# TinfoilHat0/Defending-Against-Backdoors-with-Robust-Learning-Rate

Hardware: NVIDIA H100
Metric: fl_rounds_per_sec (higher is better)
Workload: dtype bf16

## Files before the change

### defending-against-backdoors-with-robust-learning-rate_b200/ops/csrc/gemm.cu

```cuda
#include <cuda.h>
#include <stdlib.h>

#include "common.cuh"
#include "gemm.h"
#include "stem_gather.cuh"
#include "wgmma.cuh"

namespace rlr {

using namespace wg;

constexpr int BM = 128;
constexpr int BK = 64;
constexpr int kConsumers = 256;
constexpr int kThreads = kConsumers + 64;
constexpr int kEpiThreads = kConsumers;

template <int BN, int kOcc = 2>
struct TileCfg {
    static_assert(kOcc != 1 || BN == 128, "the one-wave configuration exists for the 128-wide tile");
    static constexpr int kStages = kOcc == 1 ? 6 : kOcc == 3 ? (BN == 64 ? 3 : 2) : (BN == 64 ? 4 : 3);
    static constexpr int kABytes = BM * BK * 2;
    static constexpr int kBBytes = BN * BK * 2;
    static constexpr int kStageBytes = kABytes + kBBytes;
// ... 3 lines not shown
    static_assert(kStagingBytes + 2 * BN * 4 <= kRingBytes, "staging aliases the operand ring");
    static constexpr int kTailBytes = BN == 128 ? 2048 : 1024;
    static constexpr int kSmemBytes = kRingBytes + 1024  + kTailBytes;
    static_assert(kStages <= 8, "SharedTail holds eight barriers per array");
};

struct __align__(8) SharedTail {
    uint64_t full[8];
    uint64_t empty[8];
    int row_index[BM];
};
static_assert(sizeof(SharedTail) <= 640, "the bias slice starts 640 bytes into the tail");

template <int BN, bool kStats, bool kBMN, int kOcc = 2>
__global__ void __launch_bounds__(kThreads, kOcc)
umma_conv_gemm_kernel(const __grid_constant__ CUtensorMap tmA, const __grid_constant__ CUtensorMap tmB, const __grid_constant__ CUtensorMap tmC,
                       const ConvGemmParams p) {
    using Cfg = TileCfg<BN, kOcc>;
    extern __shared__ uint8_t smem_raw[];
    uint8_t* smem = reinterpret_cast<uint8_t*>((reinterpret_cast<uintptr_t>(smem_raw) + 1023) & ~uintptr_t(1023));
    SharedTail* tail = reinterpret_cast<SharedTail*>(smem + Cfg::kRingBytes);

    const int warp = threadIdx.x >> 5, lane = threadIdx.x & 31;
    const int tile_m = blockIdx.x, tile_n = blockIdx.y;
    long long* dbg = p.dbg ? p.dbg + ((size_t)blockIdx.y * gridDim.x + blockIdx.x) * 8 : nullptr;
    if (dbg && threadIdx.x == 0) { dbg[0] = (long long)gtimer(); uint32_t sm; asm volatile("mov.u32 %0, %%smid;" : "=r"(sm)); dbg[7] = sm; }

    int n0 = 0, h0 = 0, w0 = 0;
    if (p.mode == 1) {
        const int tw_i = tile_m % p.tiles_w;
        const int th_i = (tile_m / p.tiles_w) % p.tiles_h;
        const int tn_i = tile_m / (p.tiles_w * p.tiles_h);
        w0 = tw_i * p.TW; h0 = th_i * p.TH; n0 = tn_i * p.TN;
    }

    if (warp == 8 && lane == 0) {
        prefetch_tmap(&tmA);
        prefetch_tmap(&tmB);
        if (p.tma_store) prefetch_tmap(&tmC);
        for (int s = 0; s < Cfg::kStages; ++s) { mbar_init(&tail->full[s], (p.split_prod || p.b_src) ? 2 : 1); mbar_init(&tail->empty[s], 8); }
        fence_barrier_init();
    }
    if (threadIdx.x < BM) {
        const int r = threadIdx.x;
        int gi;
        if (p.mode == 1) {
            const int tw = r % p.TW, th = (r / p.TW) % p.TH, tn = r / (p.TW * p.TH);
            const int w = w0 + tw, h = h0 + th, n = n0 + tn;
            gi = (w < p.Wo && h < p.Ho && n < p.NB) ? ((n * p.OutH + h * p.out_stride + p.out_ph) * p.OutW + w * p.out_stride + p.out_pw) : -1;
        } else {
            gi = tile_m * BM + r;
            if (gi >= p.M) gi = -1;
        }
        tail->row_index[r] = gi;
    }
    __syncthreads();
    pdl_wait();
    pdl_trigger();
    if (dbg && threadIdx.x == 0) dbg[1] = (long long)gtimer();

    if (warp == 8) {
        if (p.b_src) {
            if (lane == 0) {
                mbar_expect_tx(&tail->full[0], Cfg::kABytes);
                tma_load_2d(&tmA, &tail->full[0], smem, 0, tile_m * BM);
            }
            stem_gather_b(p, smem + Cfg::kABytes, BN, tile_n, lane);
            if (lane == 0) mbar_arrive(&tail->full[0]);
        } else if (lane == 0) {
            int stage = 0;
            uint32_t phase = 0;
            for (int kb = 0; kb < p.num_kb; ++kb) {
                mbar_wait(&tail->empty[stage], phase ^ 1);
                uint8_t* sa = smem + stage * Cfg::kStageBytes;
                uint8_t* sb = sa + Cfg::kABytes;
                mbar_expect_tx(&tail->full[stage], p.split_prod ? Cfg::kABytes : Cfg::kStageBytes);
                if (dbg && kb == 0) dbg[2] = (long long)gtimer();
                if (p.mode == 1) {
                    const int tap = kb / p.cblocks, cb = kb - tap * p.cblocks;
                    tma_load_4d(&tmA, &tail->full[stage], sa, cb * BK, w0 * p.in_stride + p.dw[tap], h0 * p.in_stride + p.dh[tap],
                                n0 + p.dn[tap]);
                } else {
                    tma_load_2d(&tmA, &tail->full[stage], sa, kb * BK, tile_m * BM);
                }
                if (p.split_prod) {
                } else if (kBMN) {
                    const int tap = kb / p.cblocks, cb = kb - tap * p.cblocks;
                    for (int g = 0; g < BN / 64; ++g)
                        tma_load_2d(&tmB, &tail->full[stage], sb + g * 8192, p.wtap[tap] * p.wcols + tile_n * BN + g * 64, cb * BK);
                } else {
                    tma_load_2d(&tmB, &tail->full[stage], sb, kb * BK, tile_n * BN);
                }
                if (++stage == Cfg::kStages) { stage = 0; phase ^= 1; }
            }
        }
    } else if (warp == 9) {
        if (p.split_prod && lane == 0) {
            int stage = 0;
            uint32_t phase = 0;
            for (int kb = 0; kb < p.num_kb; ++kb) {
                mbar_wait(&tail->empty[stage], phase ^ 1);
                uint8_t* sb = smem + stage * Cfg::kStageBytes + Cfg::kABytes;
                mbar_expect_tx(&tail->full[stage], Cfg::kBBytes);
                if (kBMN) {
                    const int tap = kb / p.cblocks, cb = kb - tap * p.cblocks;
                    for (int g = 0; g < BN / 64; ++g)
                        tma_load_2d(&tmB, &tail->full[stage], sb + g * 8192, p.wtap[tap] * p.wcols + tile_n * BN + g * 64, cb * BK);
                } else {
                    tma_load_2d(&tmB, &tail->full[stage], sb, kb * BK, tile_n * BN);
                }
                if (++stage == Cfg::kStages) { stage = 0; phase ^= 1; }
            }
        }
    } else {
        const int et = threadIdx.x;
        const int wgi = et >> 7, t = et & 127;
        const int col0 = tile_n * BN;
        const bool has_bias = !kBMN && p.bias != nullptr;
        float* bias_w = reinterpret_cast<float*>(reinterpret_cast<uint8_t*>(tail) + 640);
        if (has_bias)
            for (int i = et; i < BN; i += kEpiThreads) bias_w[i] = (col0 + i < p.N) ? p.bias[col0 + i] : 0.f;
        float acc[BN / 2];
#pragma unroll
        for (int i = 0; i < BN / 2; ++i) acc[i] = 0.f;
        {
            int stage = 0;
            uint32_t phase = 0;
            consumer_mainloop<BN, Cfg::kStages, Cfg::kStageBytes, Cfg::kABytes, kBMN>(
                acc, smem, tail->full, tail->empty, p.num_kb, (uint32_t)wgi * 64 * 128, p.b_src ? smem_u32(smem + Cfg::kABytes) : 0u,
                stage, phase, lane);
        }
        if (dbg && et == 0) dbg[4] = (long long)gtimer();
        named_bar(1, kEpiThreads);
        if (dbg && et == 0) dbg[5] = (long long)gtimer();
        const float* bias_s = bias_w;
        uint8_t* staging = smem;
        float* red = reinterpret_cast<float*>(staging + Cfg::kStagingBytes);
        const int r0 = wgi * 64 + frag_row(t, 0);
        int gi_r[2];
        gi_r[0] = tail->row_index[r0];
        gi_r[1] = tail->row_index[r0 + 8];
        if (kStats) {
            for (int i = et; i < 2 * BN; i += kEpiThreads) red[i] = 0.f;
            named_bar(1, kEpiThreads);
        }
        const bool tma_out = !kStats && p.tma_store;
#pragma unroll
        for (int j = 0; j < BN / 8; ++j) {
            const int c = frag_col(t, 4 * j);
            float s1[2] = {0.f, 0.f}, s2[2] = {0.f, 0.f};
#pragma unroll
            for (int h = 0; h < 2; ++h) {
// ... 145 lines not shown
}

template <int BN>
cudaError_t launch_persistent_bn(const CUtensorMap& tmA, const CUtensorMap& tmB, const ConvGemmParams& p, int m_tiles, int num_sms,
                                 cudaStream_t st, int occ = 1);

static int g_occ3 = -1;
void set_conv_occ3(int level) { g_occ3 = level < 0 ? 0 : (level > 1 ? 1 : level); }
static int conv_occ3() {
    if (g_occ3 < 0) { const char* e = getenv("RLR_CONV_OCC3"); set_conv_occ3(e ? atoi(e) : 1); }
    return g_occ3;
}

template <int BN, int kOcc>
static cudaError_t launch_bn_occ(const CUtensorMap& tmA, const CUtensorMap& tmB, const CUtensorMap& tmC, const ConvGemmParams& p, int m_tiles,
                                 cudaStream_t st) {
    using Cfg = TileCfg<BN, kOcc>;
    static bool configured = false;
    if (!configured) {
        RLR_CUDA_CHECK(cudaFuncSetAttribute(umma_conv_gemm_kernel<BN, false, false, kOcc>, cudaFuncAttributeMaxDynamicSharedMemorySize, Cfg::kSmemBytes));
        RLR_CUDA_CHECK(cudaFuncSetAttribute(umma_conv_gemm_kernel<BN, false, true, kOcc>, cudaFuncAttributeMaxDynamicSharedMemorySize, Cfg::kSmemBytes));
        configured = true;
    }
    dim3 grid(m_tiles, (p.N + BN - 1) / BN);
    if (p.b_mn) return launch_kernel(umma_conv_gemm_kernel<BN, false, true, kOcc>, grid, dim3(kThreads), Cfg::kSmemBytes, st, tmA, tmB, tmC, p);
    return launch_kernel(umma_conv_gemm_kernel<BN, false, false, kOcc>, grid, dim3(kThreads), Cfg::kSmemBytes, st, tmA, tmB, tmC, p);
}

static int sm_count() {
    static const int sms = [] {
        int dev = 0, n = 0;
        if (cudaGetDevice(&dev) != cudaSuccess || cudaDeviceGetAttribute(&n, cudaDevAttrMultiProcessorCount, dev) != cudaSuccess) return 132;
        return n;
    }();
    return sms;
}

static int g_persistent = -1;
void set_persistent_conv(int on) { g_persistent = on ? 1 : 0; }

static int persistent_sms() {
    if (g_persistent < 0) { const char* e = getenv("RLR_PERSISTENT_CONV"); g_persistent = (e && atoi(e) > 0) ? 1 : 0; }
    if (!g_persistent) return 0;
    static const int sms = [] {
        int dev = 0, n = 0;
        if (cudaGetDevice(&dev) != cudaSuccess || cudaDeviceGetAttribute(&n, cudaDevAttrMultiProcessorCount, dev) != cudaSuccess) return 0;
        return n;
// ... 14 lines not shown
    return g_tma_store != 0;
}
static cudaError_t make_out_tmap(CUtensorMap* tmC, const ConvGemmParams& p) {
    if (p.ldc % 8) return cudaErrorInvalidValue;
    if (p.mode == 1) {
        const uint64_t d[4] = {(uint64_t)p.N, (uint64_t)p.Wo, (uint64_t)p.Ho, (uint64_t)p.NB};
        const uint64_t s[3] = {(uint64_t)p.out_stride * p.ldc * 2, (uint64_t)p.out_stride * p.OutW * p.ldc * 2, (uint64_t)p.OutH * p.OutW * p.ldc * 2};
        const uint32_t b[4] = {64, (uint32_t)p.TW, (uint32_t)p.TH, (uint32_t)p.TN};
        const char* base = reinterpret_cast<const char*>(p.out) + ((size_t)p.out_ph * p.OutW + p.out_pw) * p.ldc * 2;
        return make_tmap_bf16(tmC, base, 4, d, s, b);
    }
    const uint64_t d[2] = {(uint64_t)p.N, (uint64_t)p.M}, s[1] = {(uint64_t)p.ldc * 2};
    const uint32_t b[2] = {64, BM};
    return make_tmap_bf16(tmC, p.out, 2, d, s, b);
}

static void finish_params(ConvGemmParams& p, CUtensorMap& tmC) {
    p.dbg = g_trace;
    {
        static const int epi_slots = [] { const char* e = getenv("RLR_EPI_STAT_SLOTS"); int v = e ? atoi(e) : 2; return v < 1 ? 1 : (v > kStatSlots ? kStatSlots : v); }();
        p.stat_slots = epi_slots;
    }
    p.tma_store = 0;
    if (tma_store_enabled() && !p.accumulate && ((reinterpret_cast<uintptr_t>(p.out) & 15) == 0) && make_out_tmap(&tmC, p) == cudaSuccess)
        p.tma_store = 1;
    if (g_split_prod < 0) { const char* e = getenv("RLR_SPLIT_PRODUCER"); g_split_prod = (e && atoi(e) == 0) ? 0 : 1; }
    p.split_prod = (g_split_prod && !p.b_src) ? 1 : 0;
}

template <int BN>
static cudaError_t launch_bn(const CUtensorMap& tmA, const CUtensorMap& tmB, const CUtensorMap& tmC, const ConvGemmParams& p, int m_tiles,
                             cudaStream_t st) {
    using Cfg = TileCfg<BN>;
    if (p.b_src && !p.stats && p.N <= BN) {
        static const int stem_persistent = [] { const char* e = getenv("RLR_STEM_PERSISTENT"); return e ? atoi(e) : 2; }();
        if (stem_persistent && m_tiles >= 2 * sm_count())
            return launch_persistent_bn<BN>(tmA, tmB, p, m_tiles, sm_count(), st, stem_persistent == 2 ? 2 : 1);
    }
    if (!p.stats && !p.b_src && persistent_sms() > 0 && m_tiles * ((p.N + BN - 1) / BN) > persistent_sms())
        return launch_persistent_bn<BN>(tmA, tmB, p, m_tiles, persistent_sms(), st);
    if constexpr (BN == 64)
        if ((!p.stats || p.tma_store) && conv_occ3() >= 1) return launch_bn_occ<BN, 3>(tmA, tmB, tmC, p, m_tiles, st);
    static bool configured = false;
    if (!configured) {
        RLR_CUDA_CHECK(cudaFuncSetAttribute(umma_conv_gemm_kernel<BN, false, false>, cudaFuncAttributeMaxDynamicSharedMemorySize, Cfg::kSmemBytes));
        RLR_CUDA_CHECK(cudaFuncSetAttribute(umma_conv_gemm_kernel<BN, true, false>, cudaFuncAttributeMaxDynamicSharedMemorySize, Cfg::kSmemBytes));
        RLR_CUDA_CHECK(cudaFuncSetAttribute(umma_conv_gemm_kernel<BN, false, true>, cudaFuncAttributeMaxDynamicSharedMemorySize, Cfg::kSmemBytes));
        configured = true;
    }
    dim3 grid(m_tiles, (p.N + BN - 1) / BN);
    if (p.b_mn) return launch_kernel(umma_conv_gemm_kernel<BN, false, true>, grid, dim3(kThreads), Cfg::kSmemBytes, st, tmA, tmB, tmC, p);
    if (p.stats && !p.tma_store) return launch_kernel(umma_conv_gemm_kernel<BN, true, false>, grid, dim3(kThreads), Cfg::kSmemBytes, st, tmA, tmB, tmC, p);
    return launch_kernel(umma_conv_gemm_kernel<BN, false, false>, grid, dim3(kThreads), Cfg::kSmemBytes, st, tmA, tmB, tmC, p);
}

static int pick_bn(int N) { return (N % 128 == 0) ? 128 : 64; }

static int g_one_wave = 1;
void set_conv_one_wave(int on) { g_one_wave = on ? 1 : 0; }

constexpr int kOneWaveMinKb = 24;
struct ConvTile { int bn; bool one_wave; };
static ConvTile pick_conv_tile(long long px, int m_tiles, int Cout, int num_kb, bool one_wave_ok) {
    const int sms = sm_count();
    if (g_one_wave && one_wave_ok && Cout % 128 == 0 && num_kb >= kOneWaveMinKb) {
        const int ctas = m_tiles * (Cout / 128);
        if (ctas <= sms && 10 * ctas >= 9 * sms) return {128, true};
    }
    const int bn = pick_bn(Cout);
    if (bn == 128 && ((px + BM - 1) / BM) * (Cout / 128) < sms) return {64, false};
    return {bn, false};
}

cudaError_t launch_gemm_bf16(const void* A, const void* B, void* out, int M, int N, int K, int lda, int ldb, int ldc,
                             const float* bias, int relu, int accumulate, float* stats, cudaStream_t st, const DropSpec* drop) {
    if (K % BK || N % 8 || M <= 0) return cudaErrorInvalidValue;
    if (drop && drop->thr && (accumulate || stats || ldc % 8)) return cudaErrorInvalidValue;
    const int m_tiles = (M + BM - 1) / BM;
    int bn = pick_bn(N);
    {
        static const int small64 = [] { const char* e = getenv("RLR_GEMM_SMALL_BN64"); return e ? atoi(e) : 0; }();
        if (small64 && bn == 128 && m_tiles * (N / 128) < sm_count()) bn = 64;
// ... 23 lines not shown
                                  cudaStream_t st) {
    if (N % 8 || M <= 0 || kvalid < 1 || kvalid > BK || ldw < kvalid) return cudaErrorInvalidValue;
    if (wait_flags && (!wait_epoch || wait_lo > wait_hi || wait_lo < 0)) return cudaErrorInvalidValue;
    const int m_tiles = (M + BM - 1) / BM;
    const int bn = pick_bn(N);
    CUtensorMap tmA;
    {
        const uint64_t d[2] = {(uint64_t)BK, (uint64_t)M}, s[1] = {(uint64_t)BK * 2};
        const uint32_t b[2] = {BK, BM};
        RLR_CUDA_CHECK(make_tmap_bf16(&tmA, A, 2, d, s, b));
    }
    ConvGemmParams p{};
    p.M = M; p.N = N; p.num_kb = 1; p.mode = 0; p.in_stride = 1; p.out_stride = 1;
    p.out = out; p.ldc = N; p.bias = bias; p.stats = stats; p.relu = relu; p.accumulate = 0;
    p.b_src = reinterpret_cast<const __nv_bfloat16*>(W); p.b_ld = ldw; p.b_kvalid = kvalid;
    p.wait_flags = wait_flags; p.wait_lo = wait_lo; p.wait_hi = wait_hi; p.wait_epoch = wait_epoch;
    CUtensorMap tmC = tmA;
    finish_params(p, tmC);
    return bn == 128 ? launch_bn<128>(tmA, tmA, tmC, p, m_tiles, st) : launch_bn<64>(tmA, tmA, tmC, p, m_tiles, st);
}

static int pow2_ceil(int x) { int p = 1; while (p < x) p <<= 1; return p; }

cudaError_t launch_conv_bf16(const void* x, const void* w, void* out, int NB, int planes, int Hin, int Win, int Cin, int Ho, int Wo,
                             int Cout, int ldc, int ntaps, const int* dh, const int* dw, const int* dplane, const float* bias,
                             int relu, int accumulate, float* stats, cudaStream_t st, const int* wtap, int w_taps_total,
                             int in_stride, int out_stride, int out_ph, int out_pw) {
    if (Cin % BK || Cout % 8 || ntaps < 1 || ntaps > 9) return cudaErrorInvalidValue;
    if (in_stride < 1 || in_stride > 2 || out_stride < 1 || out_stride > 2 || (in_stride > 1 && planes != 1)) return cudaErrorInvalidValue;
    if (wtap && (stats || Cout % 64)) return cudaErrorInvalidValue;
    ConvGemmParams p{};
    int TW = pow2_ceil(Wo); if (TW > BM) TW = BM;
    int TH = pow2_ceil(Ho); if (TW * TH > BM) TH = BM / TW;
    int TN = BM / (TW * TH);
    p.TW = TW; p.TH = TH; p.TN = TN;
    p.tiles_w = (Wo + TW - 1) / TW; p.tiles_h = (Ho + TH - 1) / TH;
    const int tiles_n = (NB + TN - 1) / TN;
    const int m_tiles = p.tiles_w * p.tiles_h * tiles_n;
    p.M = NB * Ho * Wo; p.N = Cout; p.mode = 1; p.cblocks = Cin / BK; p.num_kb = ntaps * p.cblocks; p.ntaps = ntaps;
    p.Ho = Ho; p.Wo = Wo; p.NB = NB;
    p.in_stride = in_stride; p.out_stride = out_stride; p.out_ph = out_ph; p.out_pw = out_pw; p.OutH = Ho * out_stride; p.OutW = Wo * out_stride;
    for (int t = 0; t < ntaps; ++t) { p.dh[t] = (int8_t)dh[t]; p.dw[t] = (int8_t)dw[t]; p.dn[t] = dplane[t] * NB; }
    p.out = out; p.ldc = ldc; p.bias = bias; p.stats = stats; p.relu = relu; p.accumulate = accumulate;
    CUtensorMap tmA, tmB, tmC{};
    finish_params(p, tmC);
    const ConvTile tile = pick_conv_tile((long long)NB * Ho * Wo, m_tiles, Cout, p.num_kb, !p.stats || p.tma_store);
    const int bn = tile.bn;
    {
        const uint64_t d[4] = {(uint64_t)Cin, (uint64_t)Win, (uint64_t)Hin, (uint64_t)planes * NB};
        const uint64_t s[3] = {(uint64_t)Cin * 2, (uint64_t)Win * Cin * 2, (uint64_t)Hin * Win * Cin * 2};
        const uint32_t b[4] = {BK, (uint32_t)TW, (uint32_t)TH, (uint32_t)TN};
        const uint32_t es[4] = {1, (uint32_t)in_stride, (uint32_t)in_stride, 1};
        RLR_CUDA_CHECK(make_tmap_bf16(&tmA, x, 4, d, s, b, in_stride > 1 ? es : nullptr));
    }
    if (wtap) {
        if (bias) return cudaErrorInvalidValue;
        p.b_mn = 1; p.wcols = Cout;
        for (int t = 0; t < ntaps; ++t) p.wtap[t] = wtap[t];
        const uint64_t cols = (uint64_t)w_taps_total * Cout;
        const uint64_t d[2] = {cols, (uint64_t)Cin}, s[1] = {cols * 2};
        const uint32_t b[2] = {64, BK};
        RLR_CUDA_CHECK(make_tmap_bf16(&tmB, w, 2, d, s, b));
    } else {
        const uint64_t K = (uint64_t)ntaps * Cin;
        const uint64_t d[2] = {K, (uint64_t)Cout}, s[1] = {K * 2};
        const uint32_t b[2] = {BK, (uint32_t)bn};
        RLR_CUDA_CHECK(make_tmap_bf16(&tmB, w, 2, d, s, b));
    }
    if (tile.one_wave) return launch_bn_occ<128, 1>(tmA, tmB, tmC, p, m_tiles, st);
    return bn == 128 ? launch_bn<128>(tmA, tmB, tmC, p, m_tiles, st) : launch_bn<64>(tmA, tmB, tmC, p, m_tiles, st);
}

}
```

### defending-against-backdoors-with-robust-learning-rate_b200/ops/csrc/gemm.h

```cpp
#pragma once
#include <cuda_runtime.h>
#include <cuda_bf16.h>
#include <stdint.h>

#include "dropspec.h"

namespace rlr {

constexpr int kStatSlots = 16;

struct ConvGemmParams {
    int M, N, num_kb;
    int mode;
    int cblocks;
    int TW, TH, TN;
    int Ho, Wo, NB;
    int tiles_w, tiles_h;
    int ntaps;
    int in_stride;
    int out_stride, out_ph, out_pw, OutH, OutW;
    int8_t dh[9], dw[9];
    int dn[9];
    int b_mn;
    int wtap[9];
    int wcols;
    DropSpec drop;
    int tma_store;
    int split_prod;
    long long* dbg;
    const __nv_bfloat16* b_src;
    int b_ld, b_kvalid;
    const uint32_t* wait_flags;
    int wait_lo, wait_hi;
    const uint32_t* wait_epoch;
    void* out;
    int ldc;
    const float* bias;
    float* stats;
    int stat_slots;
    int relu, accumulate;
};

cudaError_t launch_gemm_bf16(const void* A, const void* B, void* out, int M, int N, int K, int lda, int ldb, int ldc,
                             const float* bias, int relu, int accumulate, float* stats, cudaStream_t st, const DropSpec* drop = nullptr);
cudaError_t launch_stem_gemm_bf16(const void* A, const void* W, void* out, int M, int N, int kvalid, int ldw, const float* bias, int relu,
                                  float* stats, const uint32_t* wait_flags, int wait_lo, int wait_hi, const uint32_t* wait_epoch,
                                  cudaStream_t st);
void set_pdl(int on);
cudaError_t launch_gemm_splitk_bf16(const void* A, const void* B, void* out, float* ws, int M, int N, int K, const float* bias, int relu,
                                    int num_sms, cudaStream_t st, const DropSpec* drop = nullptr);
void set_persistent_conv(int on);
void set_conv_occ3(int level);
void set_conv_one_wave(int on);
void set_conv_tma_store(int on);
void set_conv_split_producer(int on);
void set_conv_trace(long long* buf);
long long* conv_trace_buf();
cudaError_t launch_conv_bf16(const void* x, const void* w, void* out, int NB, int planes, int Hin, int Win, int Cin, int Ho, int Wo,
                             int Cout, int ldc, int ntaps, const int* dh, const int* dw, const int* dplane, const float* bias,
                             int relu, int accumulate, float* stats, cudaStream_t st, const int* wtap = nullptr, int w_taps_total = 0,
                             int in_stride = 1, int out_stride = 1, int out_ph = 0, int out_pw = 0);

cudaError_t launch_conv3x3_halo_bf16(const void* x, const void* w, void* out, int NB, int Hin, int Win, int H, int W, int Cout, const float* bias,
                                     int relu, int accumulate, float* stats, int bo_mode, long long* dbg, int num_sms, cudaStream_t st);

cudaError_t launch_conv3x3_halo3_bf16(const void* x, const void* w, void* out, int NB, int H, int W, int Cout, const float* bias, int relu,
                                      int accumulate, int num_sms, cudaStream_t st);

cudaError_t launch_conv_wgrad_bf16(const void* dy, const void* x, float* dW, int NB, int planes, int Hin, int Win, int Cin, int Cin_valid,
                                   int Ho, int Wo, int Cout, int ntaps, const int* dh, const int* dw, const int* dplane, int num_sms,
                                   cudaStream_t st, int in_stride = 1);
cudaError_t launch_conv_wgrad_halo_bf16(const void* dy, const void* x, float* dW, int NB, int H, int W, int Cin_valid, int Cout,
                                        int num_sms, cudaStream_t st);
cudaError_t launch_linear_wgrad_bf16(const void* dy, const void* x, float* dW, int B, int N, int K, int num_sms, cudaStream_t st);

cudaError_t launch_ordered_sum_f32(float* out, const float* part, int nparts, long long n, cudaStream_t st);
cudaError_t launch_ordered_sum_f64(double* out, const double* part, int nparts, long long n, cudaStream_t st);
cudaError_t launch_channel_stats(const __nv_bfloat16* x, long long M, int C, float* stats , int num_sms, cudaStream_t st,
                                 int only_sum = 0, int nslots = 1);
cudaError_t launch_bn_finalize(const float* stats, int slots, float* mean_rstd, float* running_mean, float* running_var, int C,
                               float count, float eps, float momentum, int train, cudaStream_t st);
cudaError_t launch_bn_apply(const __nv_bfloat16* x, const __nv_bfloat16* res, __nv_bfloat16* y, const float* gamma, const float* beta,
                            float* mean_rstd, long long M, int C, int relu, int fin_mode, const float* stats, int slots, float count,
                            float eps, float momentum, float* running_mean, float* running_var, int num_sms, cudaStream_t st);
// ... 40 lines not shown
```

### defending-against-backdoors-with-robust-learning-rate_b200/ops/csrc/gemm_binding.cpp

```cpp
#include <torch/extension.h>
#include <ATen/cuda/CUDAContext.h>
#include <c10/cuda/CUDAGuard.h>
#include <c10/cuda/CUDAStream.h>
#include <c10/cuda/CUDACachingAllocator.h>

#include <vector>

#include "gemm.h"

namespace rlr {
void* scratch_alloc(size_t bytes, cudaStream_t st) {
    return c10::cuda::CUDACachingAllocator::raw_alloc_with_stream(bytes < 256 ? 256 : bytes, st);
}
void scratch_free(void* p) { c10::cuda::CUDACachingAllocator::raw_delete(p); }
}

namespace {
inline cudaStream_t cur_stream() { return c10::cuda::getCurrentCUDAStream().stream(); }
inline int num_sms() { return at::cuda::getCurrentDeviceProperties()->multiProcessorCount; }
inline void check(cudaError_t e, const char* what) { TORCH_CHECK(e == cudaSuccess, what, ": ", cudaGetErrorString(e)); }
template <typename T>
inline T* opt(const c10::optional<at::Tensor>& t) { return t.has_value() && t->defined() ? reinterpret_cast<T*>(t->data_ptr()) : nullptr; }
inline const __nv_bfloat16* bf(const at::Tensor& t) {
    TORCH_CHECK(t.is_cuda() && t.scalar_type() == at::kBFloat16 && t.is_contiguous(), "expected contiguous CUDA bf16 tensor");
// ... 66 lines not shown
    check(rlr::launch_gemm_splitk_bf16(bf(A), bf(B), bfm(out), f32(ws), M, N, K, opt<const float>(bias), relu, num_sms(), cur_stream(),
                                       drop.thr ? &drop : nullptr), "gemm_splitk_bf16");
}

void conv_bf16_strided(at::Tensor x, at::Tensor w, at::Tensor out, std::vector<int64_t> dh, std::vector<int64_t> dw,
                       c10::optional<at::Tensor> bias, bool relu, bool accumulate, std::vector<int64_t> wtap, int64_t w_taps_total,
                       int64_t in_stride, int64_t out_stride, int64_t out_ph, int64_t out_pw) {
    c10::cuda::CUDAGuard g(x.device());
    TORCH_CHECK(x.dim() == 4 && out.dim() == 4 && w.dim() == 2 && x.size(0) == out.size(0));
    TORCH_CHECK(out.size(1) % out_stride == 0 && out.size(2) % out_stride == 0, "output image must be a multiple of out_stride");
    const int NB = x.size(0), Hin = x.size(1), Win = x.size(2), Cin = x.size(3), Cout = out.size(3);
    const int Ho = out.size(1) / out_stride, Wo = out.size(2) / out_stride;
    const int T = (int)dh.size();
    const bool bmn = !wtap.empty();
    TORCH_CHECK(bmn ? (w.size(0) == Cin && w.size(1) == w_taps_total * Cout && (int)wtap.size() == T)
                    : (w.size(0) == Cout && w.size(1) == (int64_t)T * Cin), "filter shape");
    int a[9], b[9], c[9] = {0}, wt[9];
    for (int t = 0; t < T; ++t) { a[t] = (int)dh[t]; b[t] = (int)dw[t]; wt[t] = bmn ? (int)wtap[t] : 0; }
    check(rlr::launch_conv_bf16(bf(x), bf(w), bfm(out), NB, 1, Hin, Win, Cin, Ho, Wo, Cout, Cout, T, a, b, c, opt<const float>(bias), relu,
                                accumulate, nullptr, cur_stream(), bmn ? wt : nullptr, (int)w_taps_total, (int)in_stride, (int)out_stride,
                                (int)out_ph, (int)out_pw), "conv_bf16_strided");
}

void conv3x3_halo_bf16(at::Tensor x, at::Tensor w, at::Tensor out, c10::optional<at::Tensor> bias, bool relu, bool accumulate,
                       c10::optional<at::Tensor> stats, int64_t bo_mode, c10::optional<at::Tensor> dbg) {
    c10::cuda::CUDAGuard g(x.device());
    TORCH_CHECK(x.dim() == 4 && x.size(3) == 64 && out.dim() == 4 && w.dim() == 2 && w.size(1) == 9 * 64 && w.size(0) == out.size(3));
    TORCH_CHECK(out.size(0) == x.size(0) && out.size(1) - x.size(1) == out.size(2) - x.size(2), "halo conv: output = input + 2*pad - 2, pad in {0,1,2}");
    TORCH_CHECK(!stats.has_value() || !stats->defined() || stats->numel() == (int64_t)rlr::kStatSlots * 2 * out.size(3), "stats must be [STAT_SLOTS,2,Cout]");
    check(rlr::launch_conv3x3_halo_bf16(bf(x), bf(w), bfm(out), x.size(0), x.size(1), x.size(2), out.size(1), out.size(2), out.size(3), opt<const float>(bias), relu,
                                        accumulate, opt<float>(stats), (int)bo_mode, opt<long long>(dbg), num_sms(), cur_stream()), "conv3x3_halo_bf16");
}

void conv3x3_halo3_bf16(at::Tensor x, at::Tensor w, at::Tensor out, c10::optional<at::Tensor> bias, bool relu, bool accumulate) {
    c10::cuda::CUDAGuard g(x.device());
    TORCH_CHECK(x.dim() == 4 && x.size(3) == 64 && out.dim() == 4 && w.dim() == 2 && w.size(1) == 9 * 64 && w.size(0) == out.size(3));
    TORCH_CHECK(out.size(0) == x.size(0) && out.size(1) == x.size(1) && out.size(2) == x.size(2));
    check(rlr::launch_conv3x3_halo3_bf16(bf(x), bf(w), bfm(out), x.size(0), x.size(1), x.size(2), out.size(3), opt<const float>(bias), relu,
                                         accumulate, num_sms(), cur_stream()), "conv3x3_halo3_bf16");
}

void conv_wgrad_bf16(at::Tensor dy, at::Tensor x, at::Tensor dW, int64_t NB, int64_t planes, int64_t cin_valid, std::vector<int64_t> dh,
                     std::vector<int64_t> dw, std::vector<int64_t> dplane) {
    c10::cuda::CUDAGuard g(x.device());
    TORCH_CHECK(x.dim() == 4 && dy.dim() == 4);
    const int Hin = x.size(1), Win = x.size(2), Cin = x.size(3), Ho = dy.size(1), Wo = dy.size(2), Cout = dy.size(3);
// ... 202 lines not shown
                      bool accumulate_dx) {
    c10::cuda::CUDAGuard g(x.device());
    check(rlr::launch_linear_small_bwd(bf(x), bf(dy), bf(w), const_cast<__nv_bfloat16*>(bfo(dx)), (float*)dw.data_ptr(), opt<float>(db),
                                       x.size(0), x.size(1), w.size(0), accumulate_dx, cur_stream()), "linear_small_bwd");
}
void linear_small_fwd2(at::Tensor x, at::Tensor w, c10::optional<at::Tensor> bias, at::Tensor y, bool relu) {
    c10::cuda::CUDAGuard g(x.device());
    check(rlr::launch_linear_small_fwd2(bf(x), bf(w), opt<const float>(bias), bfm(y), x.size(0), x.size(1), w.size(0), relu, cur_stream()), "linear_small_fwd2");
}
void linear_small_bwd2(at::Tensor x, at::Tensor dy, at::Tensor w, c10::optional<at::Tensor> dx, at::Tensor dw, c10::optional<at::Tensor> db,
                       bool accumulate_dx) {
    c10::cuda::CUDAGuard g(x.device());
    check(rlr::launch_linear_small_bwd2(bf(x), bf(dy), bf(w), const_cast<__nv_bfloat16*>(bfo(dx)), (float*)dw.data_ptr(), opt<float>(db),
                                        x.size(0), x.size(1), w.size(0), accumulate_dx, cur_stream()), "linear_small_bwd2");
}
}

void register_gemm_bindings(py::module_& m) {
    m.attr("STAT_SLOTS") = rlr::kStatSlots;
    m.def("set_persistent_conv", [](bool on) { rlr::set_persistent_conv(on ? 1 : 0); });
    m.def("set_pdl", [](bool on) { rlr::set_pdl(on ? 1 : 0); });
    m.def("set_conv_occ3", [](int64_t level) { rlr::set_conv_occ3((int)level); });
    m.def("set_conv_one_wave", [](bool on) { rlr::set_conv_one_wave(on ? 1 : 0); });
    m.def("set_conv_tma_store", [](bool on) { rlr::set_conv_tma_store(on ? 1 : 0); });
    m.def("set_conv_split_producer", [](bool on) { rlr::set_conv_split_producer(on ? 1 : 0); });
    m.def("set_conv_trace", [](c10::optional<at::Tensor> buf) {
        rlr::set_conv_trace(buf.has_value() && buf->defined() ? reinterpret_cast<long long*>(buf->data_ptr<int64_t>()) : nullptr);
    });
    m.def("gemm_bf16", &gemm_bf16, py::arg("A"), py::arg("B"), py::arg("out"), py::arg("bias"), py::arg("relu"), py::arg("accumulate"), py::arg("stats"),
          py::arg("drop_p") = 0.0, py::arg("drop_seed") = 0, py::arg("drop_step") = py::none(), py::arg("drop_stream") = 0);
    m.def("stem_gemm_bf16", &stem_gemm_bf16, py::arg("A"), py::arg("W"), py::arg("out"), py::arg("bias"), py::arg("relu"), py::arg("stats"),
          py::arg("ready_ptr") = 0, py::arg("lo") = 0, py::arg("hi") = 0, py::arg("epoch") = py::none());
    m.def("gemm_splitk_bf16", &gemm_splitk_bf16, py::arg("A"), py::arg("B"), py::arg("out"), py::arg("ws"), py::arg("bias"), py::arg("relu"),
          py::arg("drop_p") = 0.0, py::arg("drop_seed") = 0, py::arg("drop_step") = py::none(), py::arg("drop_stream") = 0);
    m.def("conv_bf16", &conv_bf16);
    m.def("conv_bf16_strided", &conv_bf16_strided);
    m.def("conv_wgrad_bf16_strided", &conv_wgrad_bf16_strided);
    m.def("conv3x3_halo_bf16", &conv3x3_halo_bf16);
    m.def("conv3x3_halo3_bf16", &conv3x3_halo3_bf16);
    m.def("conv_wgrad_bf16", &conv_wgrad_bf16);
    m.def("linear_wgrad_bf16", &linear_wgrad_bf16);
    m.def("conv_wgrad_halo_bf16", &conv_wgrad_halo_bf16);
    m.def("channel_stats", &channel_stats);
    m.def("ordered_sum", &ordered_sum);
    m.def("bias_grad", &bias_grad);
    m.def("bn_finalize", &bn_finalize);
    m.def("bn_apply", &bn_apply);
    m.def("bn_bwd", &bn_bwd);
    m.def("bn_bwd_recompute", &bn_bwd_recompute);
    m.def("gn_fwd", &gn_fwd);
    m.def("gn_bwd", &gn_bwd);
    m.def("relu_bwd", &relu_bwd, py::arg("dy"), py::arg("y"), py::arg("scale") = 1.0);
    m.def("maxpool2_fwd", &maxpool2_fwd, py::arg("x"), py::arg("y"), py::arg("idx"), py::arg("drop_p") = 0.0, py::arg("drop_seed") = 0,
          py::arg("drop_step") = py::none(), py::arg("drop_stream") = 0);
    m.def("maxpool2_bwd", &maxpool2_bwd, py::arg("dy"), py::arg("idx"), py::arg("dx"), py::arg("drop_p") = 0.0, py::arg("drop_seed") = 0,
          py::arg("drop_step") = py::none(), py::arg("drop_stream") = 0, py::arg("relu_out") = py::none());
    m.def("avgpool_fwd", &avgpool_fwd);
    m.def("avgpool_bwd", &avgpool_bwd);
    m.def("dropout_fwd", &dropout_fwd);
// ... 12 lines not shown
```

### defending-against-backdoors-with-robust-learning-rate_b200/ops/nn.py

```python
from __future__ import annotations

import math
import os

import torch
import torch.nn.functional as F

_scratch = {}
_s2d_done = {}
STAT_SLOTS = 16
USE_WGRAD_HALO = True
USE_STRIDED_TMA = bool(int(os.environ.get("RLR_STRIDED_TMA", "1")))
USE_IM2COL_STEM = bool(int(os.environ.get("RLR_IM2COL_STEM", "1")))
USE_BN_RECOMPUTE = bool(int(os.environ.get("RLR_BN_RECOMPUTE", "1")))
USE_HALO3 = bool(int(os.environ.get("RLR_HALO3", "0")))
USE_HALO_ANY = bool(int(os.environ.get("RLR_HALO_ANY", "1")))
USE_SPLITK = bool(int(os.environ.get("RLR_SPLITK", "1")))
USE_HEAD_V2 = bool(int(os.environ.get("RLR_HEAD_V2", "1")))


def _stem_ok(k, stride, cin, cout):
    return USE_IM2COL_STEM and stride == 1 and cin * k * k <= 64 and cout % 8 == 0 and (cout <= 64 or cout % 128 == 0)


# ... 148 lines not shown
        return dx
    wt = scratch(("wt", w.data_ptr(), dx.data_ptr()), (Cin, k * k * Cout), w.dtype, w.device)
    e.filter_transpose(w, wt, Cout, k * k, Cin)
    e.conv_bf16(dy, wt, dx, B, 1, dh, dw, pl, None, False, bool(accumulate), None, [], 0)
    return dx


def _conv2d_dgrad_s2(e, dy, w, dx, pad, accumulate):
    Cout, k, _, Cin = w.shape
    B, Ho, Wo, _ = dy.shape
    plan = []
    for pi in range(2):
        for pj in range(2):
            taps, dh, dw = [], [], []
            for fy in range(k):
                for fx in range(k):
                    if (pi + pad - fy) % 2 == 0 and (pj + pad - fx) % 2 == 0:
                        taps.append(fy * k + fx); dh.append((pi + pad - fy) // 2); dw.append((pj + pad - fx) // 2)
            if taps:
                plan.append((pi, pj, taps, dh, dw))
    if USE_STRIDED_TMA and Cin % 64 == 0 and dx.shape[1] == 2 * Ho and dx.shape[2] == 2 * Wo:
        if not accumulate and len(plan) < 4:
            _zero(dx)
        for pi, pj, taps, dh, dw in plan:
            e.conv_bf16_strided(dy, w.reshape(Cout, k * k * Cin), dx, dh, dw, None, False, bool(accumulate), taps, k * k, 1, 2, pi, pj)
        return dx
    dx4 = scratch(("dx4", w.data_ptr(), dx.data_ptr()), (4 * B, Ho, Wo, Cin), dy.dtype, dy.device)
    mask = 0
    for pi, pj, taps, dh, dw in plan:
        plane = pi * 2 + pj
        mask |= 1 << plane
        if Cin % 64 == 0:
            e.conv_bf16(dy, w.reshape(Cout, k * k * Cin), dx4[plane * B:(plane + 1) * B], B, 1, dh, dw, [0] * len(taps), None,
                        False, False, None, taps, k * k)
            continue
        wt = scratch(("wt_s2", w.data_ptr(), dx.data_ptr(), plane), (Cin, len(taps) * Cout), w.dtype, w.device)
        e.filter_gather_transpose(w, wt, Cout, k * k, Cin, taps)
        e.conv_bf16(dy, wt, dx4[plane * B:(plane + 1) * B], B, 1, dh, dw, [0] * len(taps), None, False, False, None, [], 0)
    e.depth_to_space(dx4, dx, bool(accumulate), mask)
    return dx


def conv2d_wgrad_sm100(x, dy, gw, gb, stride, pad, tag="fwd", zero=True):
    e = _ext()
    Cout, k = gw.shape[0], gw.shape[1]
    pre = x.dim() == 2
# ... 320 lines not shown
```

Before: 0.6981.

## Merge stride-2 dgrad parity planes into one conv kernel launch

```diff
diff --git a/defending-against-backdoors-with-robust-learning-rate_b200/ops/csrc/gemm.cu b/defending-against-backdoors-with-robust-learning-rate_b200/ops/csrc/gemm.cu
--- a/defending-against-backdoors-with-robust-learning-rate_b200/ops/csrc/gemm.cu
+++ b/defending-against-backdoors-with-robust-learning-rate_b200/ops/csrc/gemm.cu
@@ -49,7 +49,13 @@
     SharedTail* tail = reinterpret_cast<SharedTail*>(smem + Cfg::kRingBytes);
 
     const int warp = threadIdx.x >> 5, lane = threadIdx.x & 31;
-    const int tile_m = blockIdx.x, tile_n = blockIdx.y;
+    const int tile_m = blockIdx.x;
+    int tile_n = blockIdx.y, num_kb = p.num_kb, tap0 = 0, out_ph = p.out_ph, out_pw = p.out_pw;
+    if (p.nplanes > 1) {
+        const int n_tiles = (p.N + BN - 1) / BN, s = blockIdx.y / n_tiles;
+        tile_n = blockIdx.y - s * n_tiles;
+        num_kb = p.plane[s].num_kb; tap0 = p.plane[s].tap0; out_ph = p.plane[s].out_ph; out_pw = p.plane[s].out_pw;
+    }
     long long* dbg = p.dbg ? p.dbg + ((size_t)blockIdx.y * gridDim.x + blockIdx.x) * 8 : nullptr;
     if (dbg && threadIdx.x == 0) { dbg[0] = (long long)gtimer(); uint32_t sm; asm volatile("mov.u32 %0, %%smid;" : "=r"(sm)); dbg[7] = sm; }
 
@@ -74,7 +80,7 @@
         if (p.mode == 1) {
             const int tw = r % p.TW, th = (r / p.TW) % p.TH, tn = r / (p.TW * p.TH);
             const int w = w0 + tw, h = h0 + th, n = n0 + tn;
-            gi = (w < p.Wo && h < p.Ho && n < p.NB) ? ((n * p.OutH + h * p.out_stride + p.out_ph) * p.OutW + w * p.out_stride + p.out_pw) : -1;
+            gi = (w < p.Wo && h < p.Ho && n < p.NB) ? ((n * p.OutH + h * p.out_stride + out_ph) * p.OutW + w * p.out_stride + out_pw) : -1;
         } else {
             gi = tile_m * BM + r;
             if (gi >= p.M) gi = -1;
@@ -97,14 +103,14 @@
         } else if (lane == 0) {
             int stage = 0;
             uint32_t phase = 0;
-            for (int kb = 0; kb < p.num_kb; ++kb) {
+            for (int kb = 0; kb < num_kb; ++kb) {
                 mbar_wait(&tail->empty[stage], phase ^ 1);
                 uint8_t* sa = smem + stage * Cfg::kStageBytes;
                 uint8_t* sb = sa + Cfg::kABytes;
                 mbar_expect_tx(&tail->full[stage], p.split_prod ? Cfg::kABytes : Cfg::kStageBytes);
                 if (dbg && kb == 0) dbg[2] = (long long)gtimer();
                 if (p.mode == 1) {
-                    const int tap = kb / p.cblocks, cb = kb - tap * p.cblocks;
+                    const int tap = tap0 + kb / p.cblocks, cb = kb - (tap - tap0) * p.cblocks;
                     tma_load_4d(&tmA, &tail->full[stage], sa, cb * BK, w0 * p.in_stride + p.dw[tap], h0 * p.in_stride + p.dh[tap],
                                 n0 + p.dn[tap]);
                 } else {
@@ -112,7 +118,7 @@
                 }
                 if (p.split_prod) {
                 } else if (kBMN) {
-                    const int tap = kb / p.cblocks, cb = kb - tap * p.cblocks;
+                    const int tap = tap0 + kb / p.cblocks, cb = kb - (tap - tap0) * p.cblocks;
                     for (int g = 0; g < BN / 64; ++g)
                         tma_load_2d(&tmB, &tail->full[stage], sb + g * 8192, p.wtap[tap] * p.wcols + tile_n * BN + g * 64, cb * BK);
                 } else {
@@ -125,12 +131,12 @@
         if (p.split_prod && lane == 0) {
             int stage = 0;
             uint32_t phase = 0;
-            for (int kb = 0; kb < p.num_kb; ++kb) {
+            for (int kb = 0; kb < num_kb; ++kb) {
                 mbar_wait(&tail->empty[stage], phase ^ 1);
                 uint8_t* sb = smem + stage * Cfg::kStageBytes + Cfg::kABytes;
                 mbar_expect_tx(&tail->full[stage], Cfg::kBBytes);
                 if (kBMN) {
-                    const int tap = kb / p.cblocks, cb = kb - tap * p.cblocks;
+                    const int tap = tap0 + kb / p.cblocks, cb = kb - (tap - tap0) * p.cblocks;
                     for (int g = 0; g < BN / 64; ++g)
                         tma_load_2d(&tmB, &tail->full[stage], sb + g * 8192, p.wtap[tap] * p.wcols + tile_n * BN + g * 64, cb * BK);
                 } else {
@@ -154,7 +160,7 @@
             int stage = 0;
             uint32_t phase = 0;
             consumer_mainloop<BN, Cfg::kStages, Cfg::kStageBytes, Cfg::kABytes, kBMN>(
-                acc, smem, tail->full, tail->empty, p.num_kb, (uint32_t)wgi * 64 * 128, p.b_src ? smem_u32(smem + Cfg::kABytes) : 0u,
+                acc, smem, tail->full, tail->empty, num_kb, (uint32_t)wgi * 64 * 128, p.b_src ? smem_u32(smem + Cfg::kABytes) : 0u,
                 stage, phase, lane);
         }
         if (dbg && et == 0) dbg[4] = (long long)gtimer();
@@ -346,7 +352,7 @@
         RLR_CUDA_CHECK(cudaFuncSetAttribute(umma_conv_gemm_kernel<BN, false, true, kOcc>, cudaFuncAttributeMaxDynamicSharedMemorySize, Cfg::kSmemBytes));
         configured = true;
     }
-    dim3 grid(m_tiles, (p.N + BN - 1) / BN);
+    dim3 grid(m_tiles, ((p.N + BN - 1) / BN) * (p.nplanes > 1 ? p.nplanes : 1));
     if (p.b_mn) return launch_kernel(umma_conv_gemm_kernel<BN, false, true, kOcc>, grid, dim3(kThreads), Cfg::kSmemBytes, st, tmA, tmB, tmC, p);
     return launch_kernel(umma_conv_gemm_kernel<BN, false, false, kOcc>, grid, dim3(kThreads), Cfg::kSmemBytes, st, tmA, tmB, tmC, p);
 }
@@ -407,7 +413,7 @@
         p.stat_slots = epi_slots;
     }
     p.tma_store = 0;
-    if (tma_store_enabled() && !p.accumulate && ((reinterpret_cast<uintptr_t>(p.out) & 15) == 0) && make_out_tmap(&tmC, p) == cudaSuccess)
+    if (tma_store_enabled() && !p.accumulate && p.nplanes <= 1 && ((reinterpret_cast<uintptr_t>(p.out) & 15) == 0) && make_out_tmap(&tmC, p) == cudaSuccess)
         p.tma_store = 1;
     if (g_split_prod < 0) { const char* e = getenv("RLR_SPLIT_PRODUCER"); g_split_prod = (e && atoi(e) == 0) ? 0 : 1; }
     p.split_prod = (g_split_prod && !p.b_src) ? 1 : 0;
@@ -422,7 +428,7 @@
         if (stem_persistent && m_tiles >= 2 * sm_count())
             return launch_persistent_bn<BN>(tmA, tmB, p, m_tiles, sm_count(), st, stem_persistent == 2 ? 2 : 1);
     }
-    if (!p.stats && !p.b_src && persistent_sms() > 0 && m_tiles * ((p.N + BN - 1) / BN) > persistent_sms())
+    if (!p.stats && !p.b_src && p.nplanes <= 1 && persistent_sms() > 0 && m_tiles * ((p.N + BN - 1) / BN) > persistent_sms())
         return launch_persistent_bn<BN>(tmA, tmB, p, m_tiles, persistent_sms(), st);
     if constexpr (BN == 64)
         if ((!p.stats || p.tma_store) && conv_occ3() >= 1) return launch_bn_occ<BN, 3>(tmA, tmB, tmC, p, m_tiles, st);
@@ -433,7 +439,7 @@
         RLR_CUDA_CHECK(cudaFuncSetAttribute(umma_conv_gemm_kernel<BN, false, true>, cudaFuncAttributeMaxDynamicSharedMemorySize, Cfg::kSmemBytes));
         configured = true;
     }
-    dim3 grid(m_tiles, (p.N + BN - 1) / BN);
+    dim3 grid(m_tiles, ((p.N + BN - 1) / BN) * (p.nplanes > 1 ? p.nplanes : 1));
     if (p.b_mn) return launch_kernel(umma_conv_gemm_kernel<BN, false, true>, grid, dim3(kThreads), Cfg::kSmemBytes, st, tmA, tmB, tmC, p);
     if (p.stats && !p.tma_store) return launch_kernel(umma_conv_gemm_kernel<BN, true, false>, grid, dim3(kThreads), Cfg::kSmemBytes, st, tmA, tmB, tmC, p);
     return launch_kernel(umma_conv_gemm_kernel<BN, false, false>, grid, dim3(kThreads), Cfg::kSmemBytes, st, tmA, tmB, tmC, p);
@@ -443,6 +449,8 @@
 
 static int g_one_wave = 1;
 void set_conv_one_wave(int on) { g_one_wave = on ? 1 : 0; }
+static int g_s2_merged = 1;
+void set_s2_dgrad_merged(int mode) { g_s2_merged = mode < 0 ? 0 : (mode > 2 ? 2 : mode); }
 
 constexpr int kOneWaveMinKb = 24;
 struct ConvTile { int bn; bool one_wave; };
@@ -512,10 +520,11 @@
 
 static int pow2_ceil(int x) { int p = 1; while (p < x) p <<= 1; return p; }
 
-cudaError_t launch_conv_bf16(const void* x, const void* w, void* out, int NB, int planes, int Hin, int Win, int Cin, int Ho, int Wo,
-                             int Cout, int ldc, int ntaps, const int* dh, const int* dw, const int* dplane, const float* bias,
-                             int relu, int accumulate, float* stats, cudaStream_t st, const int* wtap, int w_taps_total,
-                             int in_stride, int out_stride, int out_ph, int out_pw) {
+static cudaError_t launch_conv(const void* x, const void* w, void* out, int NB, int planes, int Hin, int Win, int Cin, int Ho, int Wo,
+                               int Cout, int ldc, int ntaps, const int* dh, const int* dw, const int* dplane, const float* bias,
+                               int relu, int accumulate, float* stats, cudaStream_t st, const int* wtap, int w_taps_total,
+                               int in_stride, int out_stride, int out_ph, int out_pw, int nsub, const int* sub_ntaps, const int* sub_ph,
+                               const int* sub_pw) {
     if (Cin % BK || Cout % 8 || ntaps < 1 || ntaps > 9) return cudaErrorInvalidValue;
     if (in_stride < 1 || in_stride > 2 || out_stride < 1 || out_stride > 2 || (in_stride > 1 && planes != 1)) return cudaErrorInvalidValue;
     if (wtap && (stats || Cout % 64)) return cudaErrorInvalidValue;
@@ -531,10 +540,21 @@
     p.Ho = Ho; p.Wo = Wo; p.NB = NB;
     p.in_stride = in_stride; p.out_stride = out_stride; p.out_ph = out_ph; p.out_pw = out_pw; p.OutH = Ho * out_stride; p.OutW = Wo * out_stride;
     for (int t = 0; t < ntaps; ++t) { p.dh[t] = (int8_t)dh[t]; p.dw[t] = (int8_t)dw[t]; p.dn[t] = dplane[t] * NB; }
+    int grid_planes = 1;
+    if (nsub > 1) {
+        if (nsub > 4 || stats || !wtap || out_stride != 2) return cudaErrorInvalidValue;
+        p.nplanes = grid_planes = nsub;
+        for (int i = 0, t0 = 0; i < nsub; t0 += sub_ntaps[i++]) {
+            if (sub_ntaps[i] < 1 || t0 + sub_ntaps[i] > ntaps) return cudaErrorInvalidValue;
+            p.plane[i].num_kb = sub_ntaps[i] * p.cblocks; p.plane[i].tap0 = t0; p.plane[i].out_ph = sub_ph[i]; p.plane[i].out_pw = sub_pw[i];
+            if (p.plane[i].num_kb < p.num_kb) p.num_kb = p.plane[i].num_kb;
+        }
+    }
     p.out = out; p.ldc = ldc; p.bias = bias; p.stats = stats; p.relu = relu; p.accumulate = accumulate;
     CUtensorMap tmA, tmB, tmC{};
     finish_params(p, tmC);
-    const ConvTile tile = pick_conv_tile((long long)NB * Ho * Wo, m_tiles, Cout, p.num_kb, !p.stats || p.tma_store);
+    ConvTile tile = pick_conv_tile((long long)grid_planes * NB * Ho * Wo, grid_planes * m_tiles, Cout, p.num_kb, !p.stats || p.tma_store);
+    if (nsub > 1 && g_s2_merged == 2) tile = {64, false};
     const int bn = tile.bn;
     {
         const uint64_t d[4] = {(uint64_t)Cin, (uint64_t)Win, (uint64_t)Hin, (uint64_t)planes * NB};
@@ -561,4 +581,43 @@
     return bn == 128 ? launch_bn<128>(tmA, tmB, tmC, p, m_tiles, st) : launch_bn<64>(tmA, tmB, tmC, p, m_tiles, st);
 }
 
-}
+cudaError_t launch_conv_bf16(const void* x, const void* w, void* out, int NB, int planes, int Hin, int Win, int Cin, int Ho, int Wo,
+                             int Cout, int ldc, int ntaps, const int* dh, const int* dw, const int* dplane, const float* bias,
+                             int relu, int accumulate, float* stats, cudaStream_t st, const int* wtap, int w_taps_total,
+                             int in_stride, int out_stride, int out_ph, int out_pw) {
+    return launch_conv(x, w, out, NB, planes, Hin, Win, Cin, Ho, Wo, Cout, ldc, ntaps, dh, dw, dplane, bias, relu, accumulate, stats, st,
+                       wtap, w_taps_total, in_stride, out_stride, out_ph, out_pw, 1, nullptr, nullptr, nullptr);
+}
+
+cudaError_t launch_conv_s2_dgrad_bf16(const void* dy, const void* w, void* dx, int NB, int Ho, int Wo, int Cin, int Cout, int w_taps_total,
+                                      int nplanes, const int* ntaps, const int* dh, const int* dw, const int* wtap, const int* ph,
+                                      const int* pw, int accumulate, cudaStream_t st) {
+    if (nplanes < 1 || nplanes > 4) return cudaErrorInvalidValue;
+    int total = 0;
+    for (int i = 0; i < nplanes; ++i) {
+        if (ntaps[i] < 1 || (ph[i] & ~1) || (pw[i] & ~1)) return cudaErrorInvalidValue;
+        total += ntaps[i];
+    }
+    if (total > 9) return cudaErrorInvalidValue;
+    const int zero[9] = {0};
+    if (nplanes == 1 || g_s2_merged == 0) {
+        for (int i = 0, t0 = 0; i < nplanes; t0 += ntaps[i++])
+            RLR_CUDA_CHECK(launch_conv(dy, w, dx, NB, 1, Ho, Wo, Cin, Ho, Wo, Cout, Cout, ntaps[i], dh + t0, dw + t0, zero, nullptr, 0, accumulate,
+                                       nullptr, st, wtap + t0, w_taps_total, 1, 2, ph[i], pw[i], 1, nullptr, nullptr, nullptr));
+        return cudaSuccess;
+    }
+    int order[4], first[4];
+    for (int i = 0, t0 = 0; i < nplanes; t0 += ntaps[i++]) { order[i] = i; first[i] = t0; }
+    for (int i = 1; i < nplanes; ++i)
+        for (int j = i; j > 0 && ntaps[order[j]] > ntaps[order[j - 1]]; --j) { const int s = order[j]; order[j] = order[j - 1]; order[j - 1] = s; }
+    int sdh[9], sdw[9], swt[9], sn[4], sph[4], spw[4], t = 0;
+    for (int s = 0; s < nplanes; ++s) {
+        const int i = order[s];
+        sn[s] = ntaps[i]; sph[s] = ph[i]; spw[s] = pw[i];
+        for (int k = 0; k < ntaps[i]; ++k, ++t) { sdh[t] = dh[first[i] + k]; sdw[t] = dw[first[i] + k]; swt[t] = wtap[first[i] + k]; }
+    }
+    return launch_conv(dy, w, dx, NB, 1, Ho, Wo, Cin, Ho, Wo, Cout, Cout, total, sdh, sdw, zero, nullptr, 0, accumulate, nullptr, st, swt,
+                       w_taps_total, 1, 2, 0, 0, nplanes, sn, sph, spw);
+}
+
+}
diff --git a/defending-against-backdoors-with-robust-learning-rate_b200/ops/csrc/gemm.h b/defending-against-backdoors-with-robust-learning-rate_b200/ops/csrc/gemm.h
--- a/defending-against-backdoors-with-robust-learning-rate_b200/ops/csrc/gemm.h
+++ b/defending-against-backdoors-with-robust-learning-rate_b200/ops/csrc/gemm.h
@@ -24,6 +24,8 @@
     int b_mn;
     int wtap[9];
     int wcols;
+    int nplanes;
+    struct { int num_kb, tap0, out_ph, out_pw; } plane[4];
     DropSpec drop;
     int tma_store;
     int split_prod;
@@ -52,6 +54,7 @@
 void set_persistent_conv(int on);
 void set_conv_occ3(int level);
 void set_conv_one_wave(int on);
+void set_s2_dgrad_merged(int mode);
 void set_conv_tma_store(int on);
 void set_conv_split_producer(int on);
 void set_conv_trace(long long* buf);
@@ -60,6 +63,9 @@
                              int Cout, int ldc, int ntaps, const int* dh, const int* dw, const int* dplane, const float* bias,
                              int relu, int accumulate, float* stats, cudaStream_t st, const int* wtap = nullptr, int w_taps_total = 0,
                              int in_stride = 1, int out_stride = 1, int out_ph = 0, int out_pw = 0);
+cudaError_t launch_conv_s2_dgrad_bf16(const void* dy, const void* w, void* dx, int NB, int Ho, int Wo, int Cin, int Cout, int w_taps_total,
+                                      int nplanes, const int* ntaps, const int* dh, const int* dw, const int* wtap, const int* ph,
+                                      const int* pw, int accumulate, cudaStream_t st);
 
 cudaError_t launch_conv3x3_halo_bf16(const void* x, const void* w, void* out, int NB, int Hin, int Win, int H, int W, int Cout, const float* bias,
                                      int relu, int accumulate, float* stats, int bo_mode, long long* dbg, int num_sms, cudaStream_t st);
diff --git a/defending-against-backdoors-with-robust-learning-rate_b200/ops/csrc/gemm_binding.cpp b/defending-against-backdoors-with-robust-learning-rate_b200/ops/csrc/gemm_binding.cpp
--- a/defending-against-backdoors-with-robust-learning-rate_b200/ops/csrc/gemm_binding.cpp
+++ b/defending-against-backdoors-with-robust-learning-rate_b200/ops/csrc/gemm_binding.cpp
@@ -112,6 +112,27 @@
                                 (int)out_ph, (int)out_pw), "conv_bf16_strided");
 }
 
+void conv_bf16_s2_dgrad(at::Tensor dy, at::Tensor w, at::Tensor dx, std::vector<int64_t> ph, std::vector<int64_t> pw,
+                        std::vector<std::vector<int64_t>> wtap, std::vector<std::vector<int64_t>> dh, std::vector<std::vector<int64_t>> dw,
+                        int64_t w_taps_total, bool accumulate) {
+    c10::cuda::CUDAGuard g(dy.device());
+    TORCH_CHECK(dy.dim() == 4 && dx.dim() == 4 && w.dim() == 2 && dy.size(0) == dx.size(0), "conv_bf16_s2_dgrad: shapes");
+    const int NB = dy.size(0), Ho = dy.size(1), Wo = dy.size(2), Cin = dy.size(3), Cout = dx.size(3);
+    TORCH_CHECK(dx.size(1) == 2 * Ho && dx.size(2) == 2 * Wo, "conv_bf16_s2_dgrad: dx must be [NB, 2Ho, 2Wo, C]");
+    TORCH_CHECK(w.size(0) == Cin && w.size(1) == w_taps_total * Cout, "filter shape");
+    const int P = (int)ph.size();
+    TORCH_CHECK(P >= 1 && P <= 4 && (int)pw.size() == P && (int)wtap.size() == P && (int)dh.size() == P && (int)dw.size() == P,
+                "conv_bf16_s2_dgrad: one (ph, pw, wtap, dh, dw) entry per plane, at most four");
+    int n[4], a[9], b[9], wt[9], pi[4], pj[4], t = 0;
+    for (int i = 0; i < P; ++i) {
+        TORCH_CHECK(dh[i].size() == wtap[i].size() && dw[i].size() == wtap[i].size() && t + wtap[i].size() <= 9, "conv_bf16_s2_dgrad: taps");
+        n[i] = (int)wtap[i].size(); pi[i] = (int)ph[i]; pj[i] = (int)pw[i];
+        for (size_t k = 0; k < wtap[i].size(); ++k, ++t) { a[t] = (int)dh[i][k]; b[t] = (int)dw[i][k]; wt[t] = (int)wtap[i][k]; }
+    }
+    check(rlr::launch_conv_s2_dgrad_bf16(bf(dy), bf(w), bfm(dx), NB, Ho, Wo, Cin, Cout, (int)w_taps_total, P, n, a, b, wt, pi, pj, accumulate,
+                                         cur_stream()), "conv_bf16_s2_dgrad");
+}
+
 void conv3x3_halo_bf16(at::Tensor x, at::Tensor w, at::Tensor out, c10::optional<at::Tensor> bias, bool relu, bool accumulate,
                        c10::optional<at::Tensor> stats, int64_t bo_mode, c10::optional<at::Tensor> dbg) {
     c10::cuda::CUDAGuard g(x.device());
@@ -360,6 +381,7 @@
     m.def("set_pdl", [](bool on) { rlr::set_pdl(on ? 1 : 0); });
     m.def("set_conv_occ3", [](int64_t level) { rlr::set_conv_occ3((int)level); });
     m.def("set_conv_one_wave", [](bool on) { rlr::set_conv_one_wave(on ? 1 : 0); });
+    m.def("set_s2_dgrad_merged", [](int64_t mode) { rlr::set_s2_dgrad_merged((int)mode); });
     m.def("set_conv_tma_store", [](bool on) { rlr::set_conv_tma_store(on ? 1 : 0); });
     m.def("set_conv_split_producer", [](bool on) { rlr::set_conv_split_producer(on ? 1 : 0); });
     m.def("set_conv_trace", [](c10::optional<at::Tensor> buf) {
@@ -373,6 +395,7 @@
           py::arg("drop_p") = 0.0, py::arg("drop_seed") = 0, py::arg("drop_step") = py::none(), py::arg("drop_stream") = 0);
     m.def("conv_bf16", &conv_bf16);
     m.def("conv_bf16_strided", &conv_bf16_strided);
+    m.def("conv_bf16_s2_dgrad", &conv_bf16_s2_dgrad);
     m.def("conv_wgrad_bf16_strided", &conv_wgrad_bf16_strided);
     m.def("conv3x3_halo_bf16", &conv3x3_halo_bf16);
     m.def("conv3x3_halo3_bf16", &conv3x3_halo3_bf16);
diff --git a/defending-against-backdoors-with-robust-learning-rate_b200/ops/nn.py b/defending-against-backdoors-with-robust-learning-rate_b200/ops/nn.py
--- a/defending-against-backdoors-with-robust-learning-rate_b200/ops/nn.py
+++ b/defending-against-backdoors-with-robust-learning-rate_b200/ops/nn.py
@@ -194,6 +194,10 @@
     if USE_STRIDED_TMA and Cin % 64 == 0 and dx.shape[1] == 2 * Ho and dx.shape[2] == 2 * Wo:
         if not accumulate and len(plan) < 4:
             _zero(dx)
+        if len(plan) > 1 and hasattr(e, "conv_bf16_s2_dgrad"):
+            ph, pw, taps, dh, dw = (list(c) for c in zip(*plan))
+            e.conv_bf16_s2_dgrad(dy, w.reshape(Cout, k * k * Cin), dx, ph, pw, taps, dh, dw, k * k, bool(accumulate))
+            return dx
         for pi, pj, taps, dh, dw in plan:
             e.conv_bf16_strided(dy, w.reshape(Cout, k * k * Cin), dx, dh, dw, None, False, bool(accumulate), taps, k * k, 1, 2, pi, pj)
         return dx
```

Measured after the change: 0.7072, median of 6. 1.3% higher.
